# CTPLab/Tera-MIND

Hardware: AMD Instinct MI355X
Metric: denoising steps/sec on 64x64x(2 stains x 2 z) patches (interior patch-steps/s) (higher is better)
Workload: dtype f32; 1 GPU; configs[1]: b=32 images x 1 interior 64x64 patch (P=1, 128 padded + 32 collage patches/step), rna_slc=4, rna_num=229, stain=all, DDPM T=50 schedule, f32, mode A (pad+patchify -> UNet -> DDPM update); parallelism=dp1 (independent patch batches)

## Files before the change

include/teramind_hip.h:

```cpp
#ifndef TERAMIND_HIP_H
#define TERAMIND_HIP_H

#include <stddef.h>
#include <stdint.h>

#ifdef __cplusplus
extern "C" {
#endif

#define TM_ABI_VERSION 1

enum {
  TM_OK = 0,
  TM_ERR_ARG = -1,
  TM_ERR_STATE = -2,
  TM_ERR_KEY = -3,
  TM_ERR_HIP = -4,
  TM_ERR_WORKSPACE = -5
};

enum { TM_DTYPE_F32 = 0, TM_DTYPE_BF16 = 1, TM_DTYPE_F16 = 2 };
enum { TM_SAMPLE_DDPM = 0, TM_SAMPLE_DDIM = 1 };

typedef struct tm_config {
// ... 140 lines not shown
  double executed_flops;
  double alg_bytes;
} tm_prof_stats;
int tm_profile_enable(tm_model* m, int on);
int tm_profile_collect(tm_model* m, tm_prof_stats* out);


int tm_op_to_cb8(const void* x_ncdhw, void* y_cb8, int N, int C, int Z, int H, int W, void* stream);
int tm_op_from_cb8(const void* x_cb8, void* y_ncdhw, int N, int C, int Z, int H, int W, void* stream);

int tm_op_conv_mfma(const void* x_cb8, const void* w_host, const void* bias_host, void* y_cb8,
                    int N, int Cin, int Cout, int Z, int S, int ksize, int zmode, int up2,
                    int tile_variant, void* stream);
int tm_op_conv_mfma_res(const void* x_cb8, const void* w_host, const void* bias_host, void* y_cb8, const void* res_cb8,
                        int res_half, int N, int Cin, int Cout, int Z, int S, int ksize, int zmode, int up2,
                        int tile_variant, void* stream);

int tm_op_conv_zpair_fused_f32(const void* x_cb8, const void* w_host, const void* bias_host, const void* norm_w_host,
                               const void* scale_host, const void* shift_host, const void* res_cb8, void* a2_out,
                               void* h1_out, void* a2_sep_out, int N, int Cin, int Cout, int Z, int S, int per_image,
                               int tile_variant, void* stream);

int tm_op_conv_ups_pair_f32(const void* x_cb8, const void* w_host, const void* bias_host, void* y_cb8, int N, int Cin,
                            int Cout, int Z, int S, int tile_variant, void* stream);

int tm_op_conv_xpair_f32(const void* x_cb8, const void* w_host, const void* bias_host, void* y_cb8, const void* res_cb8,
                         int res_half, int N, int Cin, int Cout, int Z, int S, int tile_variant, void* stream);
int tm_op_conv_pad1_time_f32(const void* x_cb8, const void* w_host, const void* bias_host, void* y_cb8, int N, int Cin,
                             int Cout, int S, int form, int tile_variant, int iters, float* ms_out, void* stream);

int tm_op_conv1_f32(const void* x_cb8, const void* w_host, const void* bias_host, void* y_cb8, const void* res_cb8,
                    const void* gate_cb8, int x_cbtot, int x_cb0, int gate_cbtot, int gate_cb0, int gate_half, int gelu,
                    int tile_variant, int N, int Cin, int Cout, int Z, int S, int* form_out, void* stream);
int tm_conv1_form(long vox, int ntile, int tile_variant);

int tm_conv_frag_addrs(int kernel, int half, int tw, int what, int wave, int p, int ky, int kx, int sub, int* out64);

int tm_op_conv27_bf16(const void* x_cb8, const void* w_host, const void* bias_host, void* y_cb8,
                      int N, int Cin, int Cout, int S, int dtype, int waves, const void* res_h16, void* y_h16,
                      int ups, int res_half, void* stream);
int tm_op_conv27_h16_z(const void* x_cb8, const void* w_host, const void* bias_host, void* y_cb8,
                       int N, int Cin, int Cout, int S, int dtype, int waves, const void* res_h16, void* y_h16,
                       int ups, int res_half, int Z, void* stream);

int tm_op_conv27_time(int N, int Cin, int Cout, int S, int dtype, int waves, int ups, int with_res, int fused,
                      int iters, float* ms_per_launch, void* stream);

int tm_op_conv27_fused(const void* x_cb8, const void* w_host, const void* bias_host, const void* norm_w_host,
                       const void* scale_host, const void* shift_host, void* a2_out, int N, int Cin, int Cout,
                       int S, int per_image, int dtype, int waves, void* stream);
int tm_op_conv27_fused_z(const void* x_cb8, const void* w_host, const void* bias_host, const void* norm_w_host,
                         const void* scale_host, const void* shift_host, void* a2_out, int N, int Cin, int Cout,
                         int S, int per_image, int dtype, int waves, int Z, void* stream);

int tm_op_conv1_bf16(const void* x_cb8, const void* w_host, const void* bias_host, void* y_cb8,
                     int N, int Cin, int Cout, int Z, int S, int gelu, int dtype, int waves, const void* res_h16,
                     const void* gate_h16, void* y_h16, void* stream);

int tm_op_conv1_h16_gate(const void* x_cb8, const void* w_host, const void* bias_host, void* y_cb8,
                         int N, int Cin, int Cout, int Z, int S, int gelu, int dtype, int waves, const void* res_h16,
                         const void* gate_h16, void* y_h16, int gate_half, int gate_cbtot, int gate_cb0, void* stream);

int tm_op_conv1_concat(const void* const* x_cb8, const int* cin, const int* collage, int nsrc, const void* w_host,
                       const void* bias_host, void* y_cb8, int N, int Cout, int Z, int S, int p1, int p2,
                       int dtype, int waves, void* stream);

// ... 113 lines not shown
```

tera-mind_amd/_lib.py:

```python
import ctypes as C
import os

_HERE = os.path.dirname(os.path.abspath(__file__))
LIB_PATH = os.environ.get("TM_LIB_PATH") or os.path.join(_HERE, "csrc", "libteramind_hip.so")

c_void_p, c_int, c_size_t, c_char_p, c_float = C.c_void_p, C.c_int, C.c_size_t, C.c_char_p, C.c_float
c_i64_p = C.POINTER(C.c_int64)


class TmConfig(C.Structure):
    _fields_ = [("patch_size", C.c_int32), ("rna_slc", C.c_int32), ("n_stain", C.c_int32),
                ("rna_num", C.c_int32), ("net_ch", C.c_int32), ("ch_mult", C.c_int32 * 4),
                ("embed_ch", C.c_int32), ("attn_res", C.c_int32), ("num_res_blocks", C.c_int32),
                ("vis_only", C.c_int32), ("dtype", C.c_int32)]


class TmStepCoefs(C.Structure):
    _fields_ = [("sqrt_recip_alphas_cumprod", c_float), ("sqrt_recipm1_alphas_cumprod", c_float),
                ("posterior_mean_coef1", c_float), ("posterior_mean_coef2", c_float),
                ("sigma", c_float), ("sqrt_alpha_bar_prev", c_float),
                ("sqrt_one_minus_alpha_bar_prev", c_float)]


class TmProfStats(C.Structure):
# ... 33 lines not shown
    "tm_sampler_step": (c_int, [C.POINTER(TmStepCoefs), c_void_p, c_void_p, c_void_p, c_void_p,
                                c_int, c_int, c_int, c_int, c_int, c_int, c_void_p]),
    "tm_pad_patchify": (c_int, [c_void_p, c_void_p, c_int, c_int, c_int, c_int, c_int, c_float, c_void_p]),
    "tm_gene_attn_workspace_bytes": (c_size_t, [c_void_p, c_int]),
    "tm_gene_attn": (c_int, [c_void_p, c_void_p, c_int, c_void_p, c_void_p, c_void_p, c_size_t, c_void_p]),
    "tm_gene_attn_readout_workspace_bytes": (c_size_t, [c_void_p, c_int, c_int]),
    "tm_gene_attn_readout": (c_int, [c_void_p, c_void_p, c_int, C.POINTER(C.c_int), c_int, c_void_p, c_void_p, c_void_p,
                                     c_size_t, c_void_p]),
    "tm_model_destroy": (c_int, [c_void_p]),
    "tm_gene_tile_dense": (c_int, [c_void_p, c_void_p, C.c_int64] + [c_int] * 6 + [c_void_p, c_void_p]),
    "tm_train_batch_images": (c_int, [c_void_p] + [c_int] * 5 + [c_void_p, c_void_p] + [c_int] * 4 + [c_void_p, c_void_p]),
    "tm_train_batch_genes": (c_int, [c_void_p, c_void_p, C.c_int64, c_void_p, c_void_p] + [c_int] * 4 + [c_void_p, c_void_p] +
                             [c_int] * 5 + [c_void_p, c_void_p]),
    "tm_blosc_decompress": (c_int, [c_void_p, c_size_t, c_void_p, c_size_t, C.POINTER(c_size_t)]),
    "tm_blosc_bound": (c_size_t, [c_size_t, c_int, c_int]),
    "tm_blosc_compress": (c_int, [c_void_p, c_size_t, c_int, c_int, c_void_p, c_size_t, c_void_p, c_void_p]),
    "tm_blosc_compress_tiles": (c_int, [c_void_p, c_int, C.c_int64] + [c_int] * 3 + [C.c_int64] * 2 + [c_void_p, c_void_p, c_int, c_void_p,
                                        C.c_int64, c_void_p, c_void_p]),
    "tm_blosc_frame_info": (c_int, [c_void_p, c_size_t, c_void_p]),
    "tm_blosc_decompress_dev": (c_int, [c_void_p, c_void_p, c_void_p, c_int, c_void_p, C.c_int64, c_void_p, c_void_p, c_void_p]),
    "tm_blosc_decompress_tiles": (c_int, [c_void_p, c_void_p, c_void_p, c_int, c_void_p, c_int] + [C.c_int64] * 3 + [c_void_p] * 3),
    "tm_u8_shrink2": (c_int, [c_void_p, c_int, c_int, C.c_int64, c_void_p, C.c_int64, c_void_p]),
    "tm_jpeg_encode_tiles": (c_int, [c_void_p, c_int, c_int, C.c_int64] + [c_int] * 3 + [c_void_p, C.c_int64] + [c_void_p] * 4),
    "tm_jpeg_tables": (c_int, [c_int, c_void_p, c_size_t, C.POINTER(c_size_t)]),
    "tm_ssim_planes": (c_int, [c_void_p, c_void_p] + [c_int] * 4 + [C.c_int64] * 4 + [C.POINTER(c_float), c_int, c_float, c_float, c_void_p, c_void_p]),
    "tm_avgpool2_pad": (c_int, [c_void_p] + [c_int] * 4 + [C.c_int64] * 2 + [c_void_p] + [C.c_int64] * 2 + [c_void_p]),
    "tm_profile_enable": (c_int, [c_void_p, c_int]),
    "tm_profile_collect": (c_int, [c_void_p, C.POINTER(TmProfStats)]),
    "tm_op_to_cb8": (c_int, [c_void_p, c_void_p, c_int, c_int, c_int, c_int, c_int, c_void_p]),
    "tm_op_from_cb8": (c_int, [c_void_p, c_void_p, c_int, c_int, c_int, c_int, c_int, c_void_p]),
    "tm_op_conv_mfma": (c_int, [c_void_p, c_void_p, c_void_p, c_void_p] + [c_int] * 9 + [c_void_p]),
    "tm_op_conv_mfma_res": (c_int, [c_void_p, c_void_p, c_void_p, c_void_p, c_void_p] + [c_int] * 10 + [c_void_p]),
    "tm_op_conv1_f32": (c_int, [c_void_p] * 6 + [c_int] * 12 + [C.POINTER(c_int), c_void_p]),
    "tm_conv1_form": (c_int, [C.c_long, c_int, c_int]),
    "tm_conv_frag_addrs": (c_int, [c_int] * 9 + [c_void_p]),
    "tm_op_conv27_bf16": (c_int, [c_void_p, c_void_p, c_void_p, c_void_p] + [c_int] * 6 + [c_void_p] * 2 + [c_int] * 2 + [c_void_p]),
    "tm_op_conv27_fused": (c_int, [c_void_p] * 7 + [c_int] * 7 + [c_void_p]),
    "tm_op_conv27_h16_z": (c_int, [c_void_p, c_void_p, c_void_p, c_void_p] + [c_int] * 6 + [c_void_p] * 2 + [c_int] * 3 + [c_void_p]),
    "tm_op_conv27_fused_z": (c_int, [c_void_p] * 7 + [c_int] * 8 + [c_void_p]),
    "tm_op_conv_zpair_fused_f32": (c_int, [c_void_p] * 10 + [c_int] * 7 + [c_void_p]),
    "tm_op_conv_ups_pair_f32": (c_int, [c_void_p] * 4 + [c_int] * 6 + [c_void_p]),
    "tm_op_conv_xpair_f32": (c_int, [c_void_p] * 5 + [c_int] * 7 + [c_void_p]),
    "tm_op_conv_pad1_time_f32": (c_int, [c_void_p] * 4 + [c_int] * 7 + [C.POINTER(c_float), c_void_p]),
    "tm_op_conv27_time":(c_int, [c_int] * 10 + [c_void_p, c_void_p]),
    "tm_op_conv1_bf16": (c_int, [c_void_p, c_void_p, c_void_p, c_void_p] + [c_int] * 8 + [c_void_p] * 4),
    "tm_op_conv1_h16_gate": (c_int, [c_void_p, c_void_p, c_void_p, c_void_p] + [c_int] * 8 + [c_void_p] * 3 + [c_int] * 3 + [c_void_p]),
    "tm_op_conv1_concat": (c_int, [c_void_p, c_void_p, c_void_p, c_int, c_void_p, c_void_p, c_void_p] + [c_int] * 8 + [c_void_p]),
    "tm_op_prep_h16": (c_int, [c_void_p] * 3 + [c_int] * 7 + [c_void_p, c_int, c_int, c_void_p, c_void_p, C.c_long] +
                       [c_int] * 4 + [c_void_p, c_void_p, c_int, c_void_p, c_void_p]),
    "tm_op_prep_f32": (c_int, [c_void_p] * 3 + [c_int] * 7 + [c_void_p, c_int, c_int, c_void_p, c_void_p, C.c_long] +
                       [c_int] * 4 + [c_void_p, c_void_p, c_int, c_void_p, c_void_p]),
    "tm_op_prep_form": (c_int, [c_void_p] * 3 + [c_int] * 9 + [c_void_p, c_int, c_int, c_int, c_void_p, c_void_p, C.c_long] +
                        [c_int] * 5 + [c_void_p, c_void_p, c_int, c_int, c_void_p, c_void_p]),
    "tm_op_stem": (c_int, [c_void_p] * 4 + [c_int] * 6 + [c_void_p]),
    "tm_op_head": (c_int, [c_void_p] * 4 + [c_int] * 6 + [c_void_p]),
    "tm_op_time_embed": (c_int, [c_void_p] * 7 + [c_int] * 3 + [c_void_p]),
    "tm_op_emb_all": (c_int, [c_void_p] * 4 + [c_int] * 3 + [c_void_p]),
    "tm_op_prep_train": (c_int, [c_void_p] * 5 + [c_float, c_int, c_void_p] + [c_int] * 4 + [c_void_p]),
    "tm_op_prep_bwd": (c_int, [c_void_p] * 6 + [c_float, c_int] + [c_void_p] * 4 + [c_int] * 4 + [c_void_p]),
    "tm_op_prep_train_rng": (c_int, [c_void_p] * 4 + [C.c_uint64, C.c_uint, c_float, c_int, c_void_p] + [c_int] * 4 + [c_void_p]),
    "tm_op_prep_bwd_rng": (c_int, [c_void_p] * 5 + [C.c_uint64, C.c_uint, c_float, c_int] + [c_void_p] * 4 + [c_int] * 4 + [c_void_p]),
    "tm_op_dropout_mask": (c_int, [C.c_uint64, C.c_uint, c_float, c_void_p] + [c_int] * 4 + [c_void_p]),
    "tm_op_conv_dgrad": (c_int, [c_void_p, c_void_p, c_void_p] + [c_int] * 6 + [c_void_p]),
    "tm_op_conv_wgrad": (c_int, [c_void_p, c_void_p, c_void_p, c_void_p] + [c_int] * 6 + [c_void_p]),
    "tm_conv_pack_floats": (C.c_long, [c_int] * 5),
    "tm_op_conv_pack_dev": (c_int, [c_void_p, c_void_p] + [c_int] * 5 + [c_void_p]),
# ... 60 lines not shown
```

tera-mind_amd/csrc/tm_conv_pack.cpp:

```cpp
#include "tm_conv_frag.h"
#include "tm_kernels.h"

#include <stdlib.h>
#include <string.h>

#include <vector>

namespace tmk {

int conv_form_taps(int form) {
  switch (form) {
    case CF_1X1: return 1;
    case CF_INPLANE: return 9;
    case CF_ZSKIP_UPS: case CF_PAIR_UPS: return 12;
    case CF_XPAIR: return 36;
    default: return 27;
  }
}
static bool form_ups(int form) { return form == CF_ZSKIP_UPS || form == CF_PAIR_UPS; }
size_t conv_pack_floats(int form, int Cout, int Cbi) {
  return (size_t)(form_ups(form) ? 4 : 1) * ((Cout + 63) / 64) * Cbi * conv_form_taps(form) * 512;
}
ConvW conv_w(int form, int Cout, int Cbi) {
  ConvW cw;
// ... 72 lines not shown
      o[i * 3 * k + 2 * k + t] = w0 - w1;
    }
  return o;
}
static std::vector<float> f23_rows(const float* w, size_t n) {
  std::vector<float> o(n * 36);
  for (size_t r = 0; r < n * 9; ++r) {
    const float* g = w + r * 3;
    float* u = o.data() + r * 4;
    u[0] = g[0];
    u[1] = ((g[0] + g[1]) + g[2]) * 0.5f;
    u[2] = ((g[0] - g[1]) + g[2]) * 0.5f;
    u[3] = g[2];
  }
  return o;
}

void conv_pack_host(int form, const float* w, int Cout, const int* seg_c, int nseg, float* out) {
  int Cin, Cbi;
  seg_counts(seg_c, nseg, Cin, Cbi);
  const size_t n = (size_t)Cout * Cin;
  if (form == CF_PAIR) {
    pack_taps(z_diff(w, n, 9).data(), Cout, seg_c, nseg, 27, out, true);
  } else if (form == CF_XPAIR) {
    pack_taps(f23_rows(z_diff(w, n, 9).data(), n).data(), Cout, seg_c, nseg, 36, out, true);
  } else if (form_ups(form)) {
    const size_t per = conv_pack_floats(form, Cout, Cbi) / 4;
    for (int ph = 0; ph < 4; ++ph) {
      std::vector<float> v = phase_sums(w, n, ph >> 1, ph & 1);
      if (form == CF_PAIR_UPS) v = z_diff(v.data(), n, 4);
      pack_taps(v.data(), Cout, seg_c, nseg, 12, out + ph * per, form == CF_PAIR_UPS);
    }
  } else {
    pack_taps(w, Cout, seg_c, nseg, conv_form_taps(form), out);
  }
}

void vec_pack_host(const float* v, const int* seg_c, int nseg, float* out) {
  int ci0 = 0, cb0 = 0;
  for (int s = 0; s < nseg; ++s) {
    const int nb = (seg_c[s] + 7) / 8;
    for (int c = 0; c < nb * 8; ++c) out[cb0 * 8 + c] = (c < seg_c[s]) ? v[ci0 + c] : 0.f;
    ci0 += seg_c[s];
    cb0 += nb;
  }
}

void transpose_host(const float* w, int rows, int cols, float* out) {
  for (int r = 0; r < rows; ++r)
    for (int c = 0; c < cols; ++c) out[(size_t)c * rows + r] = w[(size_t)r * cols + c];
}

void direct_pack_host(const float* w, int Cout, int Cin, int taps, float* out) {
  const int Cop = (Cout + 7) / 8 * 8;
  for (size_t i = 0; i < (size_t)taps * Cin * Cop; ++i) out[i] = 0.f;
  for (int co = 0; co < Cout; ++co)
    for (int ci = 0; ci < Cin; ++ci)
      for (int t = 0; t < taps; ++t) out[((size_t)t * Cin + ci) * Cop + co] = w[((size_t)co * Cin + ci) * taps + t];
}

}
```

tera-mind_amd/csrc/tm_kernels.hip:

```cpp
#include "tm_conv_pair.h"

#include <stdlib.h>
#include <string.h>

#include <type_traits>

namespace tmk {

template <int NZI, int WM, int TW, bool UPS = false>
struct C3Geo {
  static constexpr int TW_ = TW;
  static constexpr int MV = 4 * WM * 32;
  static constexpr int TR = (MV / TW < TW) ? (MV / TW) : TW;
  static constexpr int NPB = MV / (TR * TW);
  static constexpr int HR = TR + 2, HC = TW + 2;
  static constexpr int XV = NPB * NZI * HR * HC;
  static constexpr int XPIECES = XV * 2;
  static constexpr int PX = (XPIECES + 255) / 256;
  static constexpr int TZ = UPS ? 4 : 9;
  static constexpr int NTAP = TZ * NZI;
  static constexpr int WFLOATS = NTAP * 512;
  static constexpr int WPIECES = WFLOATS / 4;
  static constexpr int PW = (WPIECES + 255) / 256;
  static constexpr int TAPS_TOTAL = (NZI == 1) ? 9 : 3 * TZ;
// ... 621 lines not shown
    }
#pragma unroll
    for (int z = 0; z < 2; ++z) {
      f32x16 o[1][1];
      o[0][0] = acc[0][0] + acc[1 + z][0];
      asm volatile("" : "+v"(o[0][0]));
      const int ooff[1] = {ooff0 >= 0 ? ooff0 + (z * S * S + qh) * 8 : -1};
      __builtin_amdgcn_sched_barrier(0);
      conv_epilogue<1, 1>(a, o, nte, h, on, ooff, 2 * S);
    }
  } else {
#pragma unroll
    for (int p = 0; p < 3; ++p) {
      const f32x16 ev = (acc[p][0] + acc[p][1]) + acc[p][2];
      acc[p][1] = (acc[p][1] - acc[p][2]) - acc[p][3];
      acc[p][0] = ev;
      asm volatile("" : "+v"(acc[p][0]), "+v"(acc[p][1]));
    }
#pragma unroll
    for (int z = 0; z < 2; ++z)
#pragma unroll
      for (int par = 0; par < 2; ++par) {
        f32x16 o[1][1];
        o[0][0] = acc[0][par] + acc[1 + z][par];
        asm volatile("" : "+v"(o[0][0]));
        const int ooff[1] = {ooff0 >= 0 ? ooff0 + (z * S * S + par) * 8 : -1};
        __builtin_amdgcn_sched_barrier(0);
        conv_epilogue<1, 1>(a, o, nte, h, on, ooff, 2 * S);
      }
  }
}

template <int WM, int WN>
__global__ __launch_bounds__(256, 2) void conv1_mfma(ConvArgs a) {
  constexpr int MV = 4 * WM * 32;
  constexpr int KC = 4;
  constexpr int XP = KC * MV * 2 / 256;
  constexpr int NT64 = WN / 2;
  constexpr int WP = NT64 * KC * 64 * 2 / 256;
  __shared__ __attribute__((aligned(16))) float lds[NT64 * KC * 512 + KC * MV * 8];
  float* lw = lds;
  float* lx = lds + NT64 * KC * 512;

  const int tid = threadIdx.x;
  const int lane = tid & 63, wv = tid >> 6;
  const int i32 = lane & 31, h = lane >> 5;
  const int bid = xcd_swizzle(blockIdx.x, gridDim.x);
  const int nt = bid % a.ntile;
  const int mtile = bid / a.ntile;
  const long VPN = (long)a.Z * a.S * a.S;
  const long vtot = VPN * a.N;

  long xoff[XP];
  int xkc[XP];
#pragma unroll
  for (int k = 0; k < XP; ++k) {
    const int i = tid + k * 256;
    const int half = i & 1;
    const int v = (i >> 1) % MV;
    xkc[k] = (i >> 1) / MV;
    const long vg = (long)mtile * MV + v;
    long off = -1;
    if (vg < vtot) {
      const long n = vg / VPN;
      off = n * a.x_nstride + (vg - n * VPN) * 8 + half * 4;
    }
    xoff[k] = off;
  }
  const float* wsrc = a.w + (long)nt * NT64 * a.Cbi * 512;

  int xb[WM], on[WM], ooff[WM];
#pragma unroll
  for (int mt = 0; mt < WM; ++mt) {
    const int v = (wv * WM + mt) * 32 + i32;
    xb[mt] = v * 8 + 4 * h;
    const long vg = (long)mtile * MV + v;
    if (vg < vtot) {
      const long n = vg / VPN;
      on[mt] = (int)n;
      ooff[mt] = (int)((vg - n * VPN) * 8);
    } else { on[mt] = 0; ooff[mt] = -1; }
  }
  const int wb = i32 * 8 + 4 * h;

  f32x16 acc[WN][WM];
#pragma unroll
  for (int ct = 0; ct < WN; ++ct)
#pragma unroll
    for (int mt = 0; mt < WM; ++mt)
#pragma unroll
      for (int r = 0; r < 16; ++r) acc[ct][mt][r] = 0.f;

  f32x4 xr[XP], wr[WP];
  const f32x4 zero4 = {0.f, 0.f, 0.f, 0.f};
  auto load_stage = [&](int cb0) {
#pragma unroll
    for (int k = 0; k < XP; ++k) {
      const int cb = cb0 + xkc[k];
      xr[k] = (xoff[k] >= 0 && cb < a.Cbi) ? *(const f32x4*)(a.x + (long)cb * a.x_plane + xoff[k]) : zero4;
    }
#pragma unroll
    for (int k = 0; k < WP; ++k) {
      const int i = tid + k * 256;
      const int t64 = i / (KC * 128), j = i - t64 * (KC * 128);
      const int cb = cb0 + j / 128;
      wr[k] = (cb < a.Cbi) ? *(const f32x4*)(wsrc + ((long)t64 * a.Cbi + cb0) * 512 + j * 4) : zero4;
    }
  };

  load_stage(0);
  for (int cb0 = 0; cb0 < a.Cbi; cb0 += KC) {
    __syncthreads();
#pragma unroll
    for (int k = 0; k < XP; ++k) *(f32x4*)(lx + (tid + k * 256) * 4) = xr[k];
#pragma unroll
    for (int k = 0; k < WP; ++k) *(f32x4*)(lw + (tid + k * 256) * 4) = wr[k];
    __syncthreads();
    if (cb0 + KC < a.Cbi) load_stage(cb0 + KC);
#pragma unroll
    for (int kc = 0; kc < KC; ++kc) {
      f32x4 wf[WN], xf[WM];
#pragma unroll
      for (int ct = 0; ct < WN; ++ct) wf[ct] = *(const f32x4*)(lw + (ct >> 1) * (KC * 512) + kc * 512 + (ct & 1) * 256 + wb);
#pragma unroll
      for (int mt = 0; mt < WM; ++mt) xf[mt] = *(const f32x4*)(lx + kc * MV * 8 + xb[mt]);
#pragma unroll
      for (int kk = 0; kk < 4; ++kk)
#pragma unroll
        for (int ct = 0; ct < WN; ++ct)
#pragma unroll
          for (int mt = 0; mt < WM; ++mt)
            acc[ct][mt] = __builtin_amdgcn_mfma_f32_32x32x2f32(wf[ct][kk], xf[mt][kk], acc[ct][mt], 0, 0, 0);
    }
  }
  conv_epilogue<WM, WN>(a, acc, nt, h, on, ooff, 0);
}

static bool conv_fills_chip(long vox, long tiles) { return (vox / 256) * tiles >= 512; }

int conv1_form(long vox, int ntile, int tile_variant) {
  if (tile_variant == 3) return (ntile & 1) == 0 ? 3 : 0;
  const int variant = tile_variant ? tile_variant : (conv_fills_chip(vox, ntile) ? 2 : 1);
  if (variant == 2 && (ntile & 1) == 0 && conv_fills_chip(vox, ntile / 2)) return 3;
  return variant == 2 ? 2 : 1;
}

int conv_tile(int form, long ovox, int ntile, int S, int tile_variant) {
  if (S == 4) return 1;
  const long tiles = (form == CF_ZSKIP_UPS || form == CF_PAIR_UPS) ? 4L * ntile : ntile;
  const int variant = tile_variant ? tile_variant : (conv_fills_chip(ovox, tiles) ? 2 : 1);
  return variant == 2 ? 2 : 1;
}

template <void (*KERN)(ConvArgs), class G, int BLOCK = 256>
static hipError_t launch_tiled(const ConvArgs& a, long factor, hipStream_t s) {
  static DevOnce attr_once;
  if (attr_once.need()) {
    hipError_t e = hipFuncSetAttribute((const void*)KERN, hipFuncAttributeMaxDynamicSharedMemorySize, G::LDS_BYTES);
    if (e != hipSuccess) return e;
    attr_once.mark();
  }
  const long tiles = (long)(a.S / G::TW_) * (a.S / G::TR);
  const long pgs = (a.N + G::NPB - 1) / G::NPB;
  hipLaunchKernelGGL(KERN, dim3((unsigned)(pgs * tiles * factor * a.ntile)), dim3(BLOCK), G::LDS_BYTES, s, a);
  return hipGetLastError();
}
template <int MAXTW, class F>
// ... 131 lines not shown
  if (what == 0 ? (sub < 0 || sub >= NC) : what == 1 ? (sub < 0 || sub > (UPS ? 3 : 0)) : false) return -1;
  const int vt = HALF ? (wv & 1) : wv, ct0 = HALF ? (wv >> 1) : 0;
  for (int lane = 0; lane < 64; ++lane) {
    const int i32 = lane & 31, h = lane >> 5;
    int a = -1;
    if (what == 0) a = zp_wtap(UPS ? p * 4 + ky * 2 + kx : p * 9 + ky * 3 + kx, sub) + conv_w_off(ct0 * 32 + i32, 4 * h);
    else if (what == 1)
      a = lx + zp_xtap<G>(p, ky, kx) + conv_lane_of<G::TR, TW, G::PS, G::HC, G::XV>(vt * 32 + conv_lane_voxel(TW, i32), h, sub >> 1, sub & 1).xb;
    else {
      const int i = wv * 64 + lane + ky * 256;
      if (conv_stage_row(i) < G::XV) a = lx + p * G::XV * 8 + conv_frag_off(conv_stage_row(i), conv_stage_half(i), G::XV);
    }
    out[lane] = a < 0 ? -1 : a * 4;
  }
  return 0;
}
template <int HALF, int TW>
static int xpair_frag_addrs(int what, int wv, int p, int ky, int q, int* out) {
  using G = XPGeo<HALF, TW>;
  if (p < 0 || p > 2 || q < 0 || q >= (what == 2 ? 4 : G::NQ) || ky < 0 || ky > (what == 2 ? 0 : 2)) return -1;
  const int pt = HALF ? 0 : (wv >> 1), ch = wv & 1, q0 = HALF ? (wv >> 1) * 2 : 0;
  for (int lane = 0; lane < 64; ++lane) {
    const int i32 = lane & 31, h = lane >> 5, tid = wv * 64 + lane;
    int a = -1;
    if (what == 0) a = q0 * 512 + conv_w_off(ch * 32 + i32, 4 * h) + (ky * 4 + q) * 512;
    else if (what == 1)
      a = 2 * G::WSLOT + q0 * G::XP * 8 + conv_lane_of<G::TR, G::PWD, G::HR * G::PWD, G::PWD, G::XP>(pt * 32 + i32, h, 0, 0).xb + xp_xtap<G>(p, q, ky);
    else if (tid < G::XITEMS)
      a = 2 * G::WSLOT + conv_frag_off(conv_stage_row(tid), conv_stage_half(tid), G::XP) + (p * 4 + q) * G::XP * 8;
    out[lane] = a < 0 ? -1 : a * 4;
  }
  return 0;
}
int conv_frag_addrs(int kernel, int half, int tw, int what, int wv, int p, int ky, int kx, int sub, int* out) {
  if (!out || kernel < 0 || kernel > 2 || half < 0 || half > 1 || what < 0 || what > 2 || wv < 0 || wv > 3) return -1;
#define TM_FRAG(H, T)                                                                                              \
  if (half == H && tw == T) {                                                                                      \
    if (kernel == 0) return zpair_frag_addrs<ZPGeo<H, T>, H, T, false>(what, wv, p, ky, kx, sub, out);              \
    if (kernel == 1) return zpair_frag_addrs<ZPUGeo<H, T>, H, T, true>(what, wv, p, ky, kx, sub, out);              \
  }
  TM_FRAG(1, 4) TM_FRAG(0, 8) TM_FRAG(1, 8) TM_FRAG(0, 16) TM_FRAG(1, 16) TM_FRAG(0, 32) TM_FRAG(1, 32)
#undef TM_FRAG
  if (kernel == 2 && tw == 8) return half ? xpair_frag_addrs<1, 8>(what, wv, p, ky, kx, out) : xpair_frag_addrs<0, 8>(what, wv, p, ky, kx, out);
  if (kernel == 2 && tw == 16) return half ? xpair_frag_addrs<1, 16>(what, wv, p, ky, kx, out) : xpair_frag_addrs<0, 16>(what, wv, p, ky, kx, out);
  return -1;
}

struct PrepArgs { PrepLaunch L; };
struct PrepDropArgs { PrepLaunch L; DropRng r; };
__device__ __forceinline__ DropRng rng_of(const PrepArgs&) { return DropRng{0ull, 0u, 0u}; }
__device__ __forceinline__ DropRng rng_of(const PrepDropArgs& a) { return a.r; }

__device__ __forceinline__ float sumsq8(const f32x4& a0, const f32x4& a1) {
  return a0[0] * a0[0] + a0[1] * a0[1] + a0[2] * a0[2] + a0[3] * a0[3] + a1[0] * a1[0] + a1[1] * a1[1] + a1[2] * a1[2] + a1[3] * a1[3];
}
template <int NSUB, bool CACHED, bool DRAW = false, class Args = PrepArgs, int WV = 4, int NCW = 8>
__global__ __launch_bounds__(WV * 64) void prep_kernel(Args pa) {
  constexpr bool WIDE = WV > 4;
  static_assert(!WIDE || (NSUB == 1 && CACHED && !DRAW && WV * NCW >= 4), "the wide form is a cached NSUB 1 form");
  const PrepLaunch& L = pa.L;
  const DropRng R = rng_of(pa);
  __shared__ float red[4][NSUB][64];
  const int tid = threadIdx.x, lane = tid & 63, wv = WIDE ? __builtin_amdgcn_readfirstlane(tid >> 6) : tid >> 6;
  const int S = L.S, Z = L.Z;
  const long vpn = (long)Z * S * S;
  const long vidx = (long)blockIdx.x * 64 + lane;
  const bool valid = vidx < vpn * L.N;
  int n = 0, z = 0, y = 0, x = 0;
// ... 952 lines not shown
```

tera-mind_amd/csrc/tm_ops.hip:

```cpp
#include "../../include/teramind_hip.h"
#include "tm_kernels.h"

#include <algorithm>
#include <cmath>
#include <cstdint>
#include <tuple>
#include <utility>
#include <vector>
#include <string.h>

using namespace tmk;

struct DevTmp {
  std::vector<void*> ptrs;
  std::vector<hipEvent_t> events;
  hipError_t err = hipSuccess;
  const char* what = "";
  bool ordered = false;
  hipStream_t st = nullptr;
  DevTmp() = default;
  explicit DevTmp(hipStream_t stream) : ordered(true), st(stream) { keep_pool(); }
  static void keep_pool() {
    static bool done[64] = {};
    int dev = 0;
// ... 231 lines not shown
    return rc;
  const int rc = finish((hipStream_t)stream, launch_conv_mfma(op.L, (hipStream_t)stream), "conv_xpair (fp32)");
  return rc ? rc : conv_tile(CF_XPAIR, (long)N * Z * S * S, op.L.w.ntile, S, tile_variant);
}

extern "C" int tm_op_conv_pad1_time_f32(const void* x_cb8, const void* w_host, const void* bias_host, void* y_cb8, int N, int Cin,
                                        int Cout, int S, int form, int tile_variant, int iters, float* ms_out, void* stream) {
  if (const int rc = xpair_args(x_cb8, w_host, bias_host, y_cb8, N, Cin, Cout, 2, S, tile_variant)) return rc;
  if ((form != 0 && form != 1) || iters < 1 || !ms_out) return fail(TM_ERR_ARG, "form must be 0 or 1, iters >= 1, ms_out non-null");
  const int cf = conv_pick_form(3, ZM_PAD1, 2, true, form ? ROLE_OP_XPAIR : ROLE_OP);
  if (!form && cf != CF_PAIR) return fail(TM_ERR_ARG, "the pair form is switched off (TM_CONV_ZPAIR=0)");
  ConvOp op;
  if (const int rc = conv_op(op, cf, w_host, bias_host, x_cb8, y_cb8, N, Cin, Cout, 2, S, 2, S, ZM_PAD1, tile_variant)) return rc;
  hipEvent_t e0 = op.tmp.event(), e1 = op.tmp.event();
  if (op.tmp.err) return op.tmp.report();
  hipStream_t st = (hipStream_t)stream;
  for (int i = 0; i < iters; ++i) {
    HIP_TRY(hipEventRecord(e0, st));
    HIP_TRY(launch_conv_mfma(op.L, st));
    HIP_TRY(hipEventRecord(e1, st));
    HIP_TRY(hipEventSynchronize(e1));
    HIP_TRY(hipEventElapsedTime(ms_out + i, e0, e1));
  }
  return finish(st, hipSuccess, "conv_pad1_time (fp32)");
}

static bool half_gate_ok(int S) { return S >= 2 && (S & (S - 1)) == 0; }

extern "C" int tm_conv1_form(long vox, int ntile, int tile_variant) { return conv1_form(vox, ntile, tile_variant); }
extern "C" int tm_conv_frag_addrs(int kernel, int half, int tw, int what, int wave, int p, int ky, int kx, int sub, int* out64) {
  return conv_frag_addrs(kernel, half, tw, what, wave, p, ky, kx, sub, out64);
}

extern "C" int tm_op_conv1_f32(const void* x_cb8, const void* w_host, const void* bias_host, void* y_cb8, const void* res_cb8,
                               const void* gate_cb8, int x_cbtot, int x_cb0, int gate_cbtot, int gate_cb0, int gate_half, int gelu,
                               int tile_variant, int N, int Cin, int Cout, int Z, int S, int* form_out, void* stream) {
  if (!x_cb8 || !w_host || !bias_host || !y_cb8) return fail(TM_ERR_ARG, "null argument");
  if (N < 1 || Cin < 1 || Cout < 1 || Z < 1 || S < 1) return fail(TM_ERR_ARG, "N, Cin, Cout, Z, S must be positive");
  const int Cbi = (Cin + 7) / 8, Cob = (Cout + 7) / 8;
  if (x_cb0 < 0 || x_cb0 + Cbi > x_cbtot)
    return fail(TM_ERR_ARG, "x slice: blocks [%d, %d) run past the %d blocks of the tensor", x_cb0, x_cb0 + Cbi, x_cbtot);
  if (gate_half && !gate_cb8) return fail(TM_ERR_ARG, "gate_half without a gate");
  if (gate_half && !half_gate_ok(S)) return fail(TM_ERR_ARG, "gate_half: S must be a power of two >= 2 (got %d)", S);
  if (gate_cb8 && (gate_cb0 < 0 || gate_cb0 + Cob > gate_cbtot))
    return fail(TM_ERR_ARG, "gate slice: blocks [%d, %d) run past the %d blocks of the tensor", gate_cb0, gate_cb0 + Cob, gate_cbtot);
  if (tile_variant < 0 || tile_variant > 3) return fail(TM_ERR_ARG, "tile_variant must be 0 (auto), 1, 2 or 3 (got %d)", tile_variant);
  ConvW cw = conv_w(CF_1X1, Cout, Cbi);
  const int form = conv1_form((long)N * Z * S * S, cw.ntile, tile_variant);
  if (!form) return fail(TM_ERR_ARG, "tile_variant 3 (128-cout tile) needs an even number of 64-cout tiles (got %d)", cw.ntile);
  if (form_out) *form_out = form;
  std::vector<float> pk(conv_pack_floats(CF_1X1, Cout, Cbi));
  conv_pack_host(CF_1X1, (const float*)w_host, Cout, &Cin, 1, pk.data());
  DevTmp tmp;
  std::tie(cw.w, cw.bias) = upload_conv(tmp, pk, bias_host, Cout);
  if (tmp.err) return tmp.report();
  ConvLaunch L;
  L.x = cb8_view(const_cast<void*>(x_cb8), N, x_cbtot * 8, Z, S, S).blocks(x_cb0, Cbi);
  L.w = cw;
  L.y = cb8_view(y_cb8, N, Cout, Z, S, S);
  L.tile_variant = tile_variant;
  L.flags = gelu ? EPI_GELU : 0;
  TV res = L.y, gate;
  if (res_cb8) { res.p = (float*)const_cast<void*>(res_cb8); L.res = &res; }
  if (gate_cb8) {
    const int Sg = gate_half ? S / 2 : S;
    gate = cb8_view(const_cast<void*>(gate_cb8), N, gate_cbtot * 8, Z, Sg, Sg).blocks(gate_cb0, Cob);
    L.gate = &gate;
    L.gate_half = gate_half ? 1 : 0;
  }
  return finish((hipStream_t)stream, launch_conv_mfma(L, (hipStream_t)stream), "conv1 (fp32)");
}

static int conv27_launch(ConvLaunchH& L, int N, int Cin, int Cout, int Z, int S, int waves, int ups, bool res, bool fused,
                         int res_half = 0) {
  if (Z < 1 || Z > 8) return fail(TM_ERR_ARG, "Z must be in 1 .. 8 (got %d)", Z);
  if (ups && Z != 2) return fail(TM_ERR_ARG, "upsampled-input form (ups): Z == 2 only (got Z = %d)", Z);
  if (res_half && Z != 2) return fail(TM_ERR_ARG, "half-resolution residual (res_half): Z == 2 only (got Z = %d)", Z);
  if (waves != 0 && waves != 4 && waves != 8 && waves != 9) return fail(TM_ERR_ARG, "waves must be 0 (auto), 4, 8 or 9 (lockstep 8-wave form)");
  if (fused && Cout != 64 && Cout != 128) return fail(TM_ERR_ARG, "fused epilogue needs Cout in {64, 128}");
  if (ups && (Cout % 128 || res)) return fail(TM_ERR_ARG, "upsampled-input form: Cout a multiple of 128, no residual");
  const int So = ups ? 2 * S : S;
  L.x = view_h16(nullptr, N, ((Cin + 7) / 8 + 1) / 2 * 16, Z, S, S);
  L.Cout = Cout; L.force_waves = waves; L.ups = ups;
  L.y = cb8_view(nullptr, N, Cout, Z, So, So);
  if (fused) { L.fuse_norm = 1; L.a2 = view_h16(nullptr, N, Cout, Z, So, So); }
  return TM_OK;
}
static int op_conv27_h16(const void* x_cb8, const void* w_host, const void* bias_host, void* y_cb8, int N, int Cin, int Cout,
                         int Z, int S, int dtype, int waves, const void* norm_w_host, const void* scale_host, const void* shift_host,
                         int per_image, void* a2_out, void* stream, const void* res_h16 = nullptr, void* y_h16 = nullptr,
                         int ups = 0, int res_half = 0) {
  if (!is_h16(dtype)) return fail(TM_ERR_ARG, "dtype must be TM_DTYPE_BF16 or TM_DTYPE_F16");
  const bool f16 = dtype == TM_DTYPE_F16, fused = norm_w_host != nullptr;
  if (fused && (!scale_host || !shift_host || !a2_out || per_image < 1))
    return fail(TM_ERR_ARG, "fused epilogue needs scale / shift / a2 and per_image >= 1");
  ConvLaunchH L;
  if (int rc = conv27_launch(L, N, Cin, Cout, Z, S, waves, ups, res_h16 != nullptr, fused, res_half)) return rc;
  hipStream_t st = (hipStream_t)stream;
  const int Cbi = (Cin + 7) / 8, nimg = (N + per_image - 1) / per_image;
  std::vector<uint16_t> pk(ups ? conv_bf16_pack_ups_elems(Cout, Cbi) : conv_bf16_pack_elems(Cout, Cbi));
  if (ups) (f16 ? conv_f16_pack_ups_host : conv_bf16_pack_ups_host)((const float*)w_host, Cout, &Cin, 1, pk.data());
  else (f16 ? conv_f16_pack_host : conv_bf16_pack_host)((const float*)w_host, Cout, &Cin, 1, pk.data());
  DevTmp tmp;
// ... 1189 lines not shown
```

tera-mind_amd/csrc/tm_train.hip:

```cpp
#include "tm_conv_frag.h"
#include "tm_device.h"

#include <algorithm>
#include <atomic>

namespace tmk {

struct PrepBwdArgs {
  const float* x; long x_ns;
  const float* g; long g_ns;
  const float* mask; long mask_ns;
  float drop_scale;
  const float* w;
  const float* scale; const float* shift; long mod_stride; int per_image;
  float* dx; long dx_ns;
  float* part_dw;
  float* part_ds; float* part_dh;
  int N, Cb, Z, S; float inv_c;
  unsigned long long drop_key; uint32_t drop_site, drop_thr;
};

template <bool DRAW>
__global__ __launch_bounds__(256) void prep_bwd_kernel(PrepBwdArgs a) {
  __shared__ float red[4][64];
// ... 424 lines not shown
}
hipError_t launch_conv_wgrad_mfma(const TV& x, const TV& dy, float* dw, int Cin, int Cout, int taps, int accumulate, float* scratch,
                                  hipStream_t s) {
  const int S = x.H, Z = x.Z;
  if ((taps != 27 && taps != 1) || x.Z != dy.Z || x.H != dy.H || x.N != dy.N || Z < 1 || Z > 4 || x.H != x.W || dy.H != dy.W || S < 1 ||
      x.N < 1 || Cin < 1 || Cout < 1 || x.Cb != (Cin + 7) / 8 || dy.Cb != (Cout + 7) / 8)
    return hipErrorInvalidValue;
  int th, tw, per;
  wgrad_tile(Z, S, th, tw);
  const int chunks = conv_wgrad_chunks(x.N, Z, S, Cin, Cout, &per);
  if (chunks > 1 && !scratch) return hipErrorInvalidValue;
  WgradMfmaArgs a{x.p, x.nstride, x.Cb, dy.p, dy.nstride, dy.Cb, chunks > 1 ? scratch : dw, x.N, Z, S, Cout, Cin,
                  x.N * ((S + th - 1) / th) * ((S + tw - 1) / tw), per, accumulate};
  const dim3 grid((unsigned)((Cout + 31) / 32), (unsigned)((Cin + 31) / 32), (unsigned)chunks);
#define TM_WGRAD(TAPS, TH, TW) hipLaunchKernelGGL((conv_wgrad_mfma_kernel<TAPS, TH, TW>), grid, dim3(256), 0, s, a)
  if (taps == 27) {
    if (th == 8) TM_WGRAD(27, 8, 8); else if (tw == 8) TM_WGRAD(27, 4, 8); else TM_WGRAD(27, 4, 4);
  } else {
    if (th == 8) TM_WGRAD(1, 8, 8); else if (tw == 8) TM_WGRAD(1, 4, 8); else TM_WGRAD(1, 4, 4);
  }
#undef TM_WGRAD
  if (chunks > 1) {
    const long nw = (long)Cout * Cin * taps;
    hipLaunchKernelGGL(conv_wgrad_reduce_kernel, dim3((unsigned)((nw + 255) / 256)), dim3(256), 0, s, scratch, nw, chunks, dw, accumulate);
  }
  return hipGetLastError();
}

__global__ __launch_bounds__(256) void conv_pack_kernel(const float* w, float* out, int Cout, int Cin, int taps, int role, int form,
                                                        long total) {
  const long i = (long)blockIdx.x * 256 + threadIdx.x;
  if (i >= total) return;
  const int Co = role ? Cin : Cout, Ci = role ? Cout : Cin, Cbi = (Ci + 7) / 8;
  const int c8 = form == CF_PAIR ? (int)(((i >> 8) & 1) * 4 + (i & 3)) : (int)(i & 7);
  const int col = form == CF_PAIR ? (int)((i >> 2) & 63) : (int)((i >> 3) & 63);
  static_assert(conv_w_off(63, 7) == 511 && conv_w_off(5, 6) == 256 + 5 * 4 + 2, "the decode above inverts conv_w_off");
  long r = i >> 9;
  const int t = (int)(r % taps); r /= taps;
  const int cb = (int)(r % Cbi), nt = (int)(r / Cbi);
  const int co = nt * 64 + col, ci = cb * 8 + c8;
  float v = 0.f;
  if (co < Co && ci < Ci) {
    const float* src = role ? w + ((long)ci * Cin + co) * taps : w + ((long)co * Cin + ci) * taps;
    auto e = [&](int u) { return src[role ? taps - 1 - u : u]; };
    if (form != CF_PAIR) v = e(t);
    else {
      const int k = t % 9, g = t / 9;
      const float w1 = e(9 + k);
      v = g == 0 ? w1 : __fsub_rn(e(g == 1 ? 18 + k : k), w1);
    }
  }
  out[i] = v;
}
hipError_t launch_conv_pack(const float* w, float* out, int Cout, int Cin, int form, int role, hipStream_t s) {
  if (form != CF_1X1 && form != CF_PLANES3 && form != CF_ZSKIP && form != CF_PAIR) return hipErrorInvalidValue;
  const int Co = role ? Cin : Cout, Ci = role ? Cout : Cin, taps = conv_form_taps(form);
  const long total = (long)conv_pack_floats(form, Co, (Ci + 7) / 8);
  hipLaunchKernelGGL(conv_pack_kernel, dim3((unsigned)((total + 255) / 256)), dim3(256), 0, s, w, out, Cout, Cin, taps, role, form, total);
  return hipGetLastError();
}



__global__ __launch_bounds__(256) void ew_kernel(int op, const float* a, const float* b, const float* c, float* o1, float* o2, long n) {
  for (long i = (long)blockIdx.x * 256 + threadIdx.x; i < n; i += (long)gridDim.x * 256) {
    const float av = a[i];
    switch (op) {
      case 0: o1[i] = av + b[i] * c[i]; break;
// ... 991 lines not shown
```

Measured before the change: 945.8 interior patch-steps/s.

## Pipeline 1x1 conv weights via LDS DMA with triple-buffered slots

Reworks the 1x1 MFMA conv kernel so weights go straight to LDS through DMA into three rotating slots, while activations are double-buffered through registers. The K-chunk per stage drops from 4 to 2, and the weight packing changes to the half-split layout so fragment reads avoid bank conflicts. The aim is to overlap global loads with MFMA work and drop one barrier per stage. It adds explicit waitcnt and priority scheduling plus a timing entry point, which makes correctness depend on the new pack layout being applied consistently.

```diff
diff --git a/include/teramind_hip.h b/include/teramind_hip.h
--- a/include/teramind_hip.h
+++ b/include/teramind_hip.h
@@ -196,6 +196,9 @@
 int tm_op_conv1_f32(const void* x_cb8, const void* w_host, const void* bias_host, void* y_cb8, const void* res_cb8,
                     const void* gate_cb8, int x_cbtot, int x_cb0, int gate_cbtot, int gate_cb0, int gate_half, int gelu,
                     int tile_variant, int N, int Cin, int Cout, int Z, int S, int* form_out, void* stream);
+int tm_op_conv1_time_f32(const void* x_cb8, const void* w_host, const void* bias_host, void* y_cb8, const void* res_cb8,
+                         const void* gate_cb8, int x_cbtot, int x_cb0, int gate_cbtot, int gate_cb0, int gate_half, int gelu,
+                         int tile_variant, int N, int Cin, int Cout, int Z, int S, int iters, float* ms_out, void* stream);
 int tm_conv1_form(long vox, int ntile, int tile_variant);
 
 int tm_conv_frag_addrs(int kernel, int half, int tw, int what, int wave, int p, int ky, int kx, int sub, int* out64);
diff --git a/tera-mind_amd/_lib.py b/tera-mind_amd/_lib.py
--- a/tera-mind_amd/_lib.py
+++ b/tera-mind_amd/_lib.py
@@ -89,6 +89,7 @@
     "tm_op_conv_mfma": (c_int, [c_void_p, c_void_p, c_void_p, c_void_p] + [c_int] * 9 + [c_void_p]),
     "tm_op_conv_mfma_res": (c_int, [c_void_p, c_void_p, c_void_p, c_void_p, c_void_p] + [c_int] * 10 + [c_void_p]),
     "tm_op_conv1_f32": (c_int, [c_void_p] * 6 + [c_int] * 12 + [C.POINTER(c_int), c_void_p]),
+    "tm_op_conv1_time_f32": (c_int, [c_void_p] * 6 + [c_int] * 13 + [C.POINTER(c_float), c_void_p]),
     "tm_conv1_form": (c_int, [C.c_long, c_int, c_int]),
     "tm_conv_frag_addrs": (c_int, [c_int] * 9 + [c_void_p]),
     "tm_op_conv27_bf16": (c_int, [c_void_p, c_void_p, c_void_p, c_void_p] + [c_int] * 6 + [c_void_p] * 2 + [c_int] * 2 + [c_void_p]),
diff --git a/tera-mind_amd/csrc/tm_conv_pack.cpp b/tera-mind_amd/csrc/tm_conv_pack.cpp
--- a/tera-mind_amd/csrc/tm_conv_pack.cpp
+++ b/tera-mind_amd/csrc/tm_conv_pack.cpp
@@ -128,7 +128,7 @@
       pack_taps(v.data(), Cout, seg_c, nseg, 12, out + ph * per, form == CF_PAIR_UPS);
     }
   } else {
-    pack_taps(w, Cout, seg_c, nseg, conv_form_taps(form), out);
+    pack_taps(w, Cout, seg_c, nseg, conv_form_taps(form), out, form == CF_1X1);
   }
 }
 
diff --git a/tera-mind_amd/csrc/tm_kernels.hip b/tera-mind_amd/csrc/tm_kernels.hip
--- a/tera-mind_amd/csrc/tm_kernels.hip
+++ b/tera-mind_amd/csrc/tm_kernels.hip
@@ -677,15 +677,37 @@
 }
 
 template <int WM, int WN>
+struct C1Geo {
+  static constexpr int MV = 4 * WM * 32;
+  static constexpr int KC = 2;
+  static constexpr int NT64 = WN / 2;
+  static constexpr int R = 3;
+  static constexpr int WSLOT = NT64 * KC * 512;
+  static constexpr int XBUF = KC * MV * 8;
+  static constexpr int XP = KC * MV * 2 / 256;
+  static constexpr int LDS_FLOATS = R * WSLOT + 2 * XBUF;
+  static_assert(KC * 2 == 4, "a 64-cout tile of a slot is four pieces of 256 floats, one per wave");
+  static_assert(LDS_FLOATS * 4 <= 80 * 1024 && R * WSLOT * 4 <= 64 * 1024, "two workgroups per CU; DMA destinations below 64 KiB");
+};
+template <class G>
+TM_HD constexpr int c1_wtap(int kc, int ct) { return ((ct >> 1) * G::KC + kc) * 512 + conv_w_off((ct & 1) * 32, 0); }
+template <class G>
+TM_HD constexpr int c1_xtap(int kc) { return kc * G::MV * 8; }
+template <class G>
+TM_HD constexpr int c1_stage_block(int I) { return I / (2 * G::MV); }
+template <class G>
+TM_HD constexpr int c1_stage_off(int I) {
+  const int i = I % (2 * G::MV);
+  return c1_xtap<G>(c1_stage_block<G>(I)) + conv_frag_off(conv_stage_row(i), conv_stage_half(i), G::MV);
+}
+
+template <int WM, int WN>
 __global__ __launch_bounds__(256, 2) void conv1_mfma(ConvArgs a) {
-  constexpr int MV = 4 * WM * 32;
-  constexpr int KC = 4;
-  constexpr int XP = KC * MV * 2 / 256;
-  constexpr int NT64 = WN / 2;
-  constexpr int WP = NT64 * KC * 64 * 2 / 256;
-  __shared__ __attribute__((aligned(16))) float lds[NT64 * KC * 512 + KC * MV * 8];
+  using G = C1Geo<WM, WN>;
+  constexpr int MV = G::MV, KC = G::KC, XP = G::XP, NT64 = G::NT64;
+  __shared__ __attribute__((aligned(16))) float lds[G::LDS_FLOATS];
   float* lw = lds;
-  float* lx = lds + NT64 * KC * 512;
+  float* lx = lds + G::R * G::WSLOT;
 
   const int tid = threadIdx.x;
   const int lane = tid & 63, wv = tid >> 6;
@@ -697,28 +719,23 @@
   const long vtot = VPN * a.N;
 
   long xoff[XP];
-  int xkc[XP];
 #pragma unroll
   for (int k = 0; k < XP; ++k) {
-    const int i = tid + k * 256;
-    const int half = i & 1;
-    const int v = (i >> 1) % MV;
-    xkc[k] = (i >> 1) / MV;
-    const long vg = (long)mtile * MV + v;
+    const int i = (tid + k * 256) % (2 * MV);
+    const long vg = (long)mtile * MV + conv_stage_row(i);
     long off = -1;
     if (vg < vtot) {
       const long n = vg / VPN;
-      off = n * a.x_nstride + (vg - n * VPN) * 8 + half * 4;
+      off = n * a.x_nstride + (vg - n * VPN) * 8 + conv_stage_half(i) * 4;
     }
     xoff[k] = off;
   }
-  const float* wsrc = a.w + (long)nt * NT64 * a.Cbi * 512;
 
   int xb[WM], on[WM], ooff[WM];
 #pragma unroll
   for (int mt = 0; mt < WM; ++mt) {
     const int v = (wv * WM + mt) * 32 + i32;
-    xb[mt] = v * 8 + 4 * h;
+    xb[mt] = conv_frag_off(v, h, MV);
     const long vg = (long)mtile * MV + v;
     if (vg < vtot) {
       const long n = vg / VPN;
@@ -726,49 +743,70 @@
       ooff[mt] = (int)((vg - n * VPN) * 8);
     } else { on[mt] = 0; ooff[mt] = -1; }
   }
-  const int wb = i32 * 8 + 4 * h;
+  const int wb = conv_w_off(i32, 4 * h);
 
   f32x16 acc[WN][WM];
-#pragma unroll
-  for (int ct = 0; ct < WN; ++ct)
-#pragma unroll
-    for (int mt = 0; mt < WM; ++mt)
-#pragma unroll
-      for (int r = 0; r < 16; ++r) acc[ct][mt][r] = 0.f;
-
-  f32x4 xr[XP], wr[WP];
+  clear_acc(acc);
+
+  const unsigned lw_lds = (unsigned)(size_t)(__attribute__((address_space(3))) float*)lw;
+  const rsrc_words wrs = weight_rsrc<true>(a.w + (long)nt * NT64 * a.Cbi * 512, NT64 * a.Cbi * 512 * 4);
+  const int wvo = lane * 16;
+  const int wvu = __builtin_amdgcn_readfirstlane(wv);
+  auto issue_w = [&](int cb0, int slot) __attribute__((always_inline)) {
+    if (cb0 + (wvu >> 1) < a.Cbi) {
+#pragma unroll
+      for (int t64 = 0; t64 < NT64; ++t64)
+        lds_dma_piece<4, 4>(lw_lds, slot + t64 * KC * 512, (t64 * a.Cbi + cb0) * 512, 0, wvu, wvo, wrs);
+    }
+  };
+
+  f32x4 xr[XP];
   const f32x4 zero4 = {0.f, 0.f, 0.f, 0.f};
-  auto load_stage = [&](int cb0) {
+  auto load_x = [&](int cb0) __attribute__((always_inline)) {
 #pragma unroll
     for (int k = 0; k < XP; ++k) {
-      const int cb = cb0 + xkc[k];
+      const int cb = cb0 + c1_stage_block<G>(tid + k * 256);
       xr[k] = (xoff[k] >= 0 && cb < a.Cbi) ? *(const f32x4*)(a.x + (long)cb * a.x_plane + xoff[k]) : zero4;
     }
-#pragma unroll
-    for (int k = 0; k < WP; ++k) {
-      const int i = tid + k * 256;
-      const int t64 = i / (KC * 128), j = i - t64 * (KC * 128);
-      const int cb = cb0 + j / 128;
-      wr[k] = (cb < a.Cbi) ? *(const f32x4*)(wsrc + ((long)t64 * a.Cbi + cb0) * 512 + j * 4) : zero4;
-    }
   };
-
-  load_stage(0);
-  for (int cb0 = 0; cb0 < a.Cbi; cb0 += KC) {
-    __syncthreads();
-#pragma unroll
-    for (int k = 0; k < XP; ++k) *(f32x4*)(lx + (tid + k * 256) * 4) = xr[k];
-#pragma unroll
-    for (int k = 0; k < WP; ++k) *(f32x4*)(lw + (tid + k * 256) * 4) = wr[k];
-    __syncthreads();
-    if (cb0 + KC < a.Cbi) load_stage(cb0 + KC);
+  auto store_x = [&](int buf) __attribute__((always_inline)) {
+#pragma unroll
+    for (int k = 0; k < XP; ++k) *(f32x4*)(lx + buf + c1_stage_off<G>(tid + k * 256)) = xr[k];
+  };
+
+  int w0 = 0, w1 = G::WSLOT, w2 = 2 * G::WSLOT;
+  int x0 = 0;
+  load_x(0);
+  issue_w(0, w0);
+  asm volatile("s_waitcnt vmcnt(0)" ::: "memory");
+  store_x(x0);
+  if (KC < a.Cbi) { load_x(KC); issue_w(KC, w1); }
+  __builtin_amdgcn_s_waitcnt(0xC07F);
+  asm volatile("" ::: "memory");
+  __builtin_amdgcn_s_barrier();
+  asm volatile("" ::: "memory");
+  auto stage = [&](int cb0, auto n1_c, auto n2_c) __attribute__((always_inline)) {
+    constexpr bool n1 = decltype(n1_c)::value, n2 = decltype(n2_c)::value;
+    if (n1) {
+      asm volatile("s_waitcnt vmcnt(0)" ::: "memory");
+      store_x(G::XBUF - x0);
+    }
+    if (n2) {
+      load_x(cb0 + 2 * KC);
+      issue_w(cb0 + 2 * KC, w2);
+    }
+    __builtin_amdgcn_sched_barrier(0);
+    const float* lwc = lw + w0 + wb;
+    const float* lxc = lx + x0;
+    __builtin_amdgcn_s_setprio(1);
 #pragma unroll
     for (int kc = 0; kc < KC; ++kc) {
+      if (!n1 && cb0 + kc >= a.Cbi) break;
       f32x4 wf[WN], xf[WM];
 #pragma unroll
-      for (int ct = 0; ct < WN; ++ct) wf[ct] = *(const f32x4*)(lw + (ct >> 1) * (KC * 512) + kc * 512 + (ct & 1) * 256 + wb);
-#pragma unroll
-      for (int mt = 0; mt < WM; ++mt) xf[mt] = *(const f32x4*)(lx + kc * MV * 8 + xb[mt]);
+      for (int ct = 0; ct < WN; ++ct) wf[ct] = *(const f32x4*)(lwc + c1_wtap<G>(kc, ct));
+#pragma unroll
+      for (int mt = 0; mt < WM; ++mt) xf[mt] = *(const f32x4*)(lxc + c1_xtap<G>(kc) + xb[mt]);
 #pragma unroll
       for (int kk = 0; kk < 4; ++kk)
 #pragma unroll
@@ -777,7 +815,22 @@
           for (int mt = 0; mt < WM; ++mt)
             acc[ct][mt] = __builtin_amdgcn_mfma_f32_32x32x2f32(wf[ct][kk], xf[mt][kk], acc[ct][mt], 0, 0, 0);
     }
-  }
+    __builtin_amdgcn_s_setprio(0);
+    if (n1) {
+      __builtin_amdgcn_s_waitcnt(0xC07F);
+      asm volatile("" ::: "memory");
+      __builtin_amdgcn_s_barrier();
+      asm volatile("" ::: "memory");
+    }
+    const int t = w0; w0 = w1; w1 = w2; w2 = t;
+    x0 = G::XBUF - x0;
+  };
+  using T = std::true_type;
+  using F = std::false_type;
+  int cb0 = 0;
+  for (; cb0 + 2 * KC < a.Cbi; cb0 += KC) stage(cb0, T{}, T{});
+  if (cb0 + KC < a.Cbi) { stage(cb0, T{}, F{}); cb0 += KC; }
+  stage(cb0, F{}, F{});
   conv_epilogue<WM, WN>(a, acc, nt, h, on, ooff, 0);
 }
 
@@ -975,8 +1028,32 @@
   }
   return 0;
 }
+template <int WM, int WN>
+static int conv1_frag_addrs(int what, int wv, int p, int ky, int kx, int sub, int* out) {
+  using G = C1Geo<WM, WN>;
+  constexpr int lx = G::R * G::WSLOT;
+  if (what == 2 ? (ky < 0 || ky >= G::XP) : (p < 0 || p >= G::KC)) return -1;
+  if (kx < 0 || kx >= (what == 0 ? G::R : 2)) return -1;
+  if (what == 0 ? (sub < 0 || sub >= WN) : what == 1 ? (sub < 0 || sub >= WM) : false) return -1;
+  for (int lane = 0; lane < 64; ++lane) {
+    const int i32 = lane & 31, h = lane >> 5;
+    int a;
+    if (what == 0) a = kx * G::WSLOT + c1_wtap<G>(p, sub) + conv_w_off(i32, 4 * h);
+    else if (what == 1) a = lx + kx * G::XBUF + c1_xtap<G>(p) + conv_frag_off((wv * WM + sub) * 32 + i32, h, G::MV);
+    else a = lx + kx * G::XBUF + c1_stage_off<G>(wv * 64 + lane + ky * 256);
+    out[lane] = a * 4;
+  }
+  return 0;
+}
 int conv_frag_addrs(int kernel, int half, int tw, int what, int wv, int p, int ky, int kx, int sub, int* out) {
-  if (!out || kernel < 0 || kernel > 2 || half < 0 || half > 1 || what < 0 || what > 2 || wv < 0 || wv > 3) return -1;
+  if (!out || kernel < 0 || kernel > 3 || half < 0 || half > 1 || what < 0 || what > 2 || wv < 0 || wv > 3) return -1;
+  if (kernel == 3) {
+    if (half) return -1;
+    if (tw == 1) return conv1_frag_addrs<1, 2>(what, wv, p, ky, kx, sub, out);
+    if (tw == 2) return conv1_frag_addrs<2, 2>(what, wv, p, ky, kx, sub, out);
+    if (tw == 3) return conv1_frag_addrs<2, 4>(what, wv, p, ky, kx, sub, out);
+    return -1;
+  }
 #define TM_FRAG(H, T)                                                                                              \
   if (half == H && tw == T) {                                                                                      \
     if (kernel == 0) return zpair_frag_addrs<ZPGeo<H, T>, H, T, false>(what, wv, p, ky, kx, sub, out);              \
diff --git a/tera-mind_amd/csrc/tm_ops.hip b/tera-mind_amd/csrc/tm_ops.hip
--- a/tera-mind_amd/csrc/tm_ops.hip
+++ b/tera-mind_amd/csrc/tm_ops.hip
@@ -287,9 +287,9 @@
   return conv_frag_addrs(kernel, half, tw, what, wave, p, ky, kx, sub, out64);
 }
 
-extern "C" int tm_op_conv1_f32(const void* x_cb8, const void* w_host, const void* bias_host, void* y_cb8, const void* res_cb8,
-                               const void* gate_cb8, int x_cbtot, int x_cb0, int gate_cbtot, int gate_cb0, int gate_half, int gelu,
-                               int tile_variant, int N, int Cin, int Cout, int Z, int S, int* form_out, void* stream) {
+static int conv1_op(const void* x_cb8, const void* w_host, const void* bias_host, void* y_cb8, const void* res_cb8,
+                    const void* gate_cb8, int x_cbtot, int x_cb0, int gate_cbtot, int gate_cb0, int gate_half, int gelu,
+                    int tile_variant, int N, int Cin, int Cout, int Z, int S, int* form_out, int iters, float* ms_out, void* stream) {
   if (!x_cb8 || !w_host || !bias_host || !y_cb8) return fail(TM_ERR_ARG, "null argument");
   if (N < 1 || Cin < 1 || Cout < 1 || Z < 1 || S < 1) return fail(TM_ERR_ARG, "N, Cin, Cout, Z, S must be positive");
   const int Cbi = (Cin + 7) / 8, Cob = (Cout + 7) / 8;
@@ -323,7 +323,31 @@
     L.gate = &gate;
     L.gate_half = gate_half ? 1 : 0;
   }
-  return finish((hipStream_t)stream, launch_conv_mfma(L, (hipStream_t)stream), "conv1 (fp32)");
+  hipStream_t st = (hipStream_t)stream;
+  if (!ms_out) return finish(st, launch_conv_mfma(L, st), "conv1 (fp32)");
+  hipEvent_t e0 = tmp.event(), e1 = tmp.event();
+  if (tmp.err) return tmp.report();
+  for (int i = 0; i < iters; ++i) {
+    HIP_TRY(hipEventRecord(e0, st));
+    HIP_TRY(launch_conv_mfma(L, st));
+    HIP_TRY(hipEventRecord(e1, st));
+    HIP_TRY(hipEventSynchronize(e1));
+    HIP_TRY(hipEventElapsedTime(ms_out + i, e0, e1));
+  }
+  return finish(st, hipSuccess, "conv1_time (fp32)");
+}
+extern "C" int tm_op_conv1_f32(const void* x_cb8, const void* w_host, const void* bias_host, void* y_cb8, const void* res_cb8,
+                               const void* gate_cb8, int x_cbtot, int x_cb0, int gate_cbtot, int gate_cb0, int gate_half, int gelu,
+                               int tile_variant, int N, int Cin, int Cout, int Z, int S, int* form_out, void* stream) {
+  return conv1_op(x_cb8, w_host, bias_host, y_cb8, res_cb8, gate_cb8, x_cbtot, x_cb0, gate_cbtot, gate_cb0, gate_half, gelu, tile_variant,
+                  N, Cin, Cout, Z, S, form_out, 1, nullptr, stream);
+}
+extern "C" int tm_op_conv1_time_f32(const void* x_cb8, const void* w_host, const void* bias_host, void* y_cb8, const void* res_cb8,
+                                    const void* gate_cb8, int x_cbtot, int x_cb0, int gate_cbtot, int gate_cb0, int gate_half, int gelu,
+                                    int tile_variant, int N, int Cin, int Cout, int Z, int S, int iters, float* ms_out, void* stream) {
+  if (iters < 1 || !ms_out) return fail(TM_ERR_ARG, "iters >= 1, ms_out non-null");
+  return conv1_op(x_cb8, w_host, bias_host, y_cb8, res_cb8, gate_cb8, x_cbtot, x_cb0, gate_cbtot, gate_cb0, gate_half, gelu, tile_variant,
+                  N, Cin, Cout, Z, S, nullptr, iters, ms_out, stream);
 }
 
 static int conv27_launch(ConvLaunchH& L, int N, int Cin, int Cout, int Z, int S, int waves, int ups, bool res, bool fused,
diff --git a/tera-mind_amd/csrc/tm_train.hip b/tera-mind_amd/csrc/tm_train.hip
--- a/tera-mind_amd/csrc/tm_train.hip
+++ b/tera-mind_amd/csrc/tm_train.hip
@@ -480,8 +480,9 @@
   const long i = (long)blockIdx.x * 256 + threadIdx.x;
   if (i >= total) return;
   const int Co = role ? Cin : Cout, Ci = role ? Cout : Cin, Cbi = (Ci + 7) / 8;
-  const int c8 = form == CF_PAIR ? (int)(((i >> 8) & 1) * 4 + (i & 3)) : (int)(i & 7);
-  const int col = form == CF_PAIR ? (int)((i >> 2) & 63) : (int)((i >> 3) & 63);
+  const bool halves = form == CF_PAIR || form == CF_1X1;
+  const int c8 = halves ? (int)(((i >> 8) & 1) * 4 + (i & 3)) : (int)(i & 7);
+  const int col = halves ? (int)((i >> 2) & 63) : (int)((i >> 3) & 63);
   static_assert(conv_w_off(63, 7) == 511 && conv_w_off(5, 6) == 256 + 5 * 4 + 2, "the decode above inverts conv_w_off");
   long r = i >> 9;
   const int t = (int)(r % taps); r /= taps;
```

After: 949.5 interior patch-steps/s (median of 6 runs). About the same (+0.4%).
